# Galtvam/OthelloZero

Measured on NVIDIA B200. Metric: mcts_sims_per_sec, higher is better.
Workload: dtype bf16

## Files before the change

### othellozero_b200/csrc/oz_net.cu

```cuda
#include <cuda.h>
#include <cuda_bf16.h>
#include <stdlib.h>

#include "oz_engine.cuh"

typedef __nv_bfloat16 bf16;

namespace {

constexpr int BLOCK_M = 128;
constexpr int BLOCK_K = 64;
constexpr int UMMA_K = 16;
constexpr int STAGES = 4;
constexpr int A_STAGE_BYTES = BLOCK_M * BLOCK_K * 2;
constexpr int GEMM_THREADS = 256;
constexpr int EPI_RELU_BF16 = 0;
constexpr int EPI_HEADS = 1;
constexpr int EPI_LINEAR_BF16 = 2;
constexpr int N_PATTERNS = 19683;

struct GemmParams {
    int num_kb;
    int chunks_per_tap;
    int ntaps_x;
    int pad;
    int nb;
    int rows_per_board;
    int rows_valid;
    int split;
    int halves;
    int half_rows;
    int half_h;
    int tile_den;
    int tile_num;
    int n_tiles;
    int ldc;
    int max_count;
    unsigned long long* trace;
    unsigned a_bytes;
    const int* count;
    const float* bias;
    bf16* out;
    float* pi; float* logits; float* v;
    int nsq;
    const int* cache_idx; float* cache_pi; float* cache_v; unsigned long long* cache_tags;
};

__device__ __forceinline__ uint32_t smem_u32(const void* p) { return (uint32_t)__cvta_generic_to_shared(p); }

__device__ __forceinline__ void mbar_init(uint32_t bar, uint32_t count) {
    asm volatile("mbarrier.init.shared::cta.b64 [%0], %1;" ::"r"(bar), "r"(count) : "memory");
}
__device__ __forceinline__ void mbar_expect_tx(uint32_t bar, uint32_t bytes) {
    asm volatile("mbarrier.arrive.expect_tx.shared::cta.b64 _, [%0], %1;" ::"r"(bar), "r"(bytes) : "memory");
}
__device__ __forceinline__ void mbar_arrive(uint32_t bar) {
    asm volatile("mbarrier.arrive.shared::cta.b64 _, [%0];" ::"r"(bar) : "memory");
}
__device__ __forceinline__ bool mbar_try_wait(uint32_t bar, uint32_t parity) {
    uint32_t ok;
    asm volatile(
        "{\n\t.reg .pred p;\n\t"
        "mbarrier.try_wait.parity.shared::cta.b64 p, [%1], %2;\n\t"
        "selp.u32 %0, 1, 0, p;\n\t}"
        : "=r"(ok) : "r"(bar), "r"(parity) : "memory");
    return ok != 0;
}
__device__ __noinline__ void mbar_wait_slow(uint32_t bar, uint32_t parity) {
    unsigned long long t0 = 0;
    uint32_t spins = 0;
    while (!mbar_try_wait(bar, parity)) {
        if ((++spins & 255u) == 0) {
            unsigned long long t;
            asm volatile("mov.u64 %0, %%globaltimer;" : "=l"(t));
            if (t0 == 0) t0 = t;
            else if (t - t0 > 4000000000ull) __trap();
        }
    }
// ... 349 lines not shown
__device__ __forceinline__ void tma_load_4d_2sm(uint32_t dst, const CUtensorMap* m, uint32_t bar, int c0, int c1, int c2, int c3) {
    asm volatile(
        "cp.async.bulk.tensor.4d.cta_group::2.shared::cluster.global.mbarrier::complete_tx::bytes [%0], [%1, {%3, %4, %5, %6}], [%2];"
        ::"r"(dst), "l"(m), "r"(bar), "r"(c0), "r"(c1), "r"(c2), "r"(c3) : "memory");
}
__device__ __forceinline__ void tma_load_2d_2sm(uint32_t dst, const CUtensorMap* m, uint32_t bar, int c0, int c1) {
    asm volatile(
        "cp.async.bulk.tensor.2d.cta_group::2.shared::cluster.global.mbarrier::complete_tx::bytes [%0], [%1, {%3, %4}], [%2];"
        ::"r"(dst), "l"(m), "r"(bar), "r"(c0), "r"(c1) : "memory");
}
__device__ __forceinline__ void tmem_alloc_2sm(uint32_t dst_smem, uint32_t cols) {
    asm volatile("tcgen05.alloc.cta_group::2.sync.aligned.shared::cta.b32 [%0], %1;" ::"r"(dst_smem), "r"(cols) : "memory");
}
__device__ __forceinline__ void tmem_relinquish_2sm() {
    asm volatile("tcgen05.relinquish_alloc_permit.cta_group::2.sync.aligned;" ::: "memory");
}
__device__ __forceinline__ void tmem_dealloc_2sm(uint32_t taddr, uint32_t cols) {
    asm volatile("tcgen05.dealloc.cta_group::2.sync.aligned.b32 %0, %1;" ::"r"(taddr), "r"(cols) : "memory");
}
__device__ __forceinline__ void umma_bf16_2sm_lo(uint32_t d_tmem, uint32_t a_lo, uint32_t b_lo, uint32_t idesc, uint32_t accumulate) {
    asm volatile(
        "{\n\t.reg .pred p;\n\t.reg .b64 da, db;\n\t"
        "setp.ne.b32 p, %4, 0;\n\t"
        "mov.b64 da, {%1, %5};\n\t"
        "mov.b64 db, {%2, %5};\n\t"
        "tcgen05.mma.cta_group::2.kind::f16 [%0], da, db, %3, p;\n\t}"
        ::"r"(d_tmem), "r"(a_lo), "r"(b_lo), "r"(idesc), "r"(accumulate), "r"(SW128_DESC_HI) : "memory");
}
__device__ __forceinline__ void umma_commit_2sm(uint32_t bar, uint16_t cta_mask) {
    asm volatile("tcgen05.commit.cta_group::2.mbarrier::arrive::one.shared::cluster.multicast::cluster.b64 [%0], %1;"
                 ::"r"(bar), "h"(cta_mask) : "memory");
}

constexpr int STAGES2 = 6;
constexpr int B2_STAGE_BYTES = 128 * BLOCK_K * 2;
struct Gemm2Smem {
    static constexpr int OFF_A = 0;
    static constexpr int OFF_B = STAGES2 * A_STAGE_BYTES;
    static constexpr int OFF_BAR = OFF_B + STAGES2 * B2_STAGE_BYTES;
    static constexpr int OFF_TMEM = OFF_BAR + (2 * STAGES2 + 4) * 8;
    static constexpr int OFF_BIAS = OFF_TMEM + 16;
    static constexpr int BYTES = OFF_BIAS + 2 * 256 * 4;
    static constexpr int DYN_BYTES = BYTES + 1024;
};

__global__ void __cluster_dims__(2, 1, 1) __launch_bounds__(GEMM_THREADS, 1)
oz_gemm2_kernel(const __grid_constant__ CUtensorMap mapA, const __grid_constant__ CUtensorMap mapA2,
                const __grid_constant__ CUtensorMap mapB, const GemmParams p) {
    using S = Gemm2Smem;
    constexpr int BLOCK_N = 256;
    constexpr uint32_t TMEM_COLS = 2 * BLOCK_N;
    extern __shared__ uint8_t smem_raw[];
    const uint32_t raw = smem_u32(smem_raw);
    const uint32_t base = (raw + 1023u) & ~1023u;
    uint8_t* gbase = smem_raw + (base - raw);
    const uint32_t sA = base + S::OFF_A, sB = base + S::OFF_B, sBar = base + S::OFF_BAR;
    auto full_bar = [&](int s) { return sBar + 8u * s; };
    auto empty_bar = [&](int s) { return sBar + 8u * (STAGES2 + s); };
    auto tfull_bar = [&](int a) { return sBar + 8u * (2 * STAGES2 + a); };
    auto tempty_bar = [&](int a) { return sBar + 8u * (2 * STAGES2 + 2 + a); };
    volatile uint32_t* s_tmem = (volatile uint32_t*)(gbase + S::OFF_TMEM);
    float* s_bias = (float*)(gbase + S::OFF_BIAS);

    const int warp = threadIdx.x >> 5, lane = threadIdx.x & 31;
    const uint32_t rank = cluster_ctarank();
    const int cluster_id = blockIdx.x >> 1, num_clusters = gridDim.x >> 1;
    trace_begin(p.trace);
    int L = *p.count;
    if (L > p.max_count) L = p.max_count;
    const int m_tiles = (L * p.tile_num + p.tile_den - 1) / p.tile_den;
    const int num_pair_tiles = ((m_tiles + 1) >> 1) * p.n_tiles;

    if (warp == 0 && lane == 0) {
        tma_prefetch_desc(&mapA);
        tma_prefetch_desc(&mapB);
    }
    if (warp == 1 && lane == 0) {
// ... 67 lines not shown
                const uint32_t d_tmem = tmem_base + (uint32_t)(acc * BLOCK_N);
                for (int kb = 0; kb < p.num_kb; ++kb) {
                    mbar_wait(full_bar(stage), phase);
                    tc_fence_after();
                    const uint32_t a_lo = a_lo0 + (uint32_t)stage * (A_STAGE_BYTES >> 4);
                    const uint32_t b_lo = b_lo0 + (uint32_t)stage * (B2_STAGE_BYTES >> 4);
                    if (elect_one()) {
#pragma unroll
                        for (int k = 0; k < BLOCK_K / UMMA_K; ++k)
                            umma_bf16_2sm_lo(d_tmem, a_lo + 2u * k, b_lo + 2u * k, idesc, (kb | k) ? 1u : 0u);
                        umma_commit_2sm(empty_bar(stage), 3);
                    }
                    __syncwarp();
                    if (++stage == STAGES2) { stage = 0; phase ^= 1u; }
                }
                if (elect_one()) umma_commit_2sm(tfull_bar(acc), 3);
                __syncwarp();
                if (++acc == 2) { acc = 0; acc_phase ^= 1u; }
            }
        }
        __syncwarp();
    } else if (warp >= 4) {
        const int ew = warp - 4;
        const int et = threadIdx.x - 128;
        int acc = 0; uint32_t acc_phase = 0;
        for (int pt = cluster_id; pt < num_pair_tiles; pt += num_clusters) {
            const int m_pair = pt / p.n_tiles, n_idx = pt - m_pair * p.n_tiles;
            const int m_tile = 2 * m_pair + (int)rank;
            float* bias = s_bias + acc * BLOCK_N;
            for (int i = et; i < BLOCK_N; i += 128) bias[i] = p.bias[n_idx * BLOCK_N + i];
            epi_bar_sync();
            mbar_wait(tfull_bar(acc), acc_phase);
            tc_fence_after();
            const int r = ew * 32 + lane;
            const long long grow = (long long)m_tile * p.rows_valid + r;
            const bool ok = (r < p.rows_valid) && (grow < (long long)L * p.rows_per_board);
            const uint32_t t_row = tmem_base + (uint32_t)(acc * BLOCK_N) + ((uint32_t)(ew * 32) << 16);
            bf16* orow = p.out + grow * p.ldc + (long long)n_idx * BLOCK_N;
#pragma unroll 1
            for (int c = 0; c < BLOCK_N / 32; ++c) {
                uint32_t v[32];
                tmem_ld32(t_row + (uint32_t)(c * 32), v);
                tmem_ld_wait();
                if (ok) {
                    uint32_t packed[16];
#pragma unroll
                    for (int j = 0; j < 16; ++j) {
                        const float2 bj = *reinterpret_cast<const float2*>(bias + c * 32 + 2 * j);
                        const float2 y = __fadd2_rn(make_float2(__uint_as_float(v[2 * j]), __uint_as_float(v[2 * j + 1])), bj);
                        packed[j] = pack_relu_bf16x2(y.x, y.y);
                    }
                    uint4* dst = reinterpret_cast<uint4*>(orow + c * 32);
#pragma unroll
                    for (int q = 0; q < 4; ++q)
                        dst[q] = make_uint4(packed[4 * q], packed[4 * q + 1], packed[4 * q + 2], packed[4 * q + 3]);
                }
            }
            tc_fence_before();
            __syncwarp();
            if (lane == 0) mbar_arrive_cluster(mapa_cluster(tempty_bar(acc), 0));
            if (++acc == 2) { acc = 0; acc_phase ^= 1u; }
        }
    }
    __syncwarp();
    tc_fence_before();
    __syncthreads();
    cluster_sync_all();
    if (warp == 2) {
        tc_fence_after();
        tmem_dealloc_2sm(tmem_base, TMEM_COLS);
    }
    trace_end(p.trace);
}

constexpr int TSTAGES = 3;
constexpr int T_B_STAGE_BYTES = 256 * BLOCK_K * 2;
struct TailSmem {
    static constexpr int OFF_A = 0;
    static constexpr int OFF_B = TSTAGES * A_STAGE_BYTES;
    static constexpr int OFF_F2 = OFF_B + TSTAGES * T_B_STAGE_BYTES;
    static constexpr int OFF_BAR = OFF_F2 + 4 * A_STAGE_BYTES;
    static constexpr int OFF_TMEM = OFF_BAR + (2 * TSTAGES + 7) * 8 + 8;
    static constexpr int OFF_BIAS = OFF_TMEM + 16;
    static constexpr int BYTES = OFF_BIAS + 640 * 4;
    static constexpr int DYN_BYTES = BYTES + 1024;
};
struct TailParams {
    int max_count;
    const int* count;
    const float* bias4; const float* bias5;
    bf16* f2;
    float* pi; float* logits; float* v;
    int nsq;
    const int* cache_idx; float* cache_pi; float* cache_v; unsigned long long* cache_tags;
    unsigned long long* trace;
    unsigned long long* dbg;
};

__global__ void __launch_bounds__(GEMM_THREADS, 1)
oz_tail_kernel(const __grid_constant__ CUtensorMap mapA ,
               const __grid_constant__ CUtensorMap mapB4 ,
               const __grid_constant__ CUtensorMap mapB5 , const TailParams p) {
    using S = TailSmem;
// ... 723 lines not shown
            Wt[(size_t)o * K + k] = __float2bfloat16(tile[threadIdx.x][i] * s);
        }
    }
    if (blockIdx.x == 0 && threadIdx.y == 0) {
        int o = o0 + threadIdx.x;
        if (o < Nout) {
            float s = gamma ? gamma[o] / sqrtf(var[o] + eps) : 1.0f;
            bias_out[o] = gamma ? (b[o] - mean[o]) * s + beta[o] : b[o];
        }
    }
}

typedef CUresult (*PFN_tmapEncodeTiled)(CUtensorMap*, CUtensorMapDataType, cuuint32_t, void*, const cuuint64_t*,
                                        const cuuint64_t*, const cuuint32_t*, const cuuint32_t*, CUtensorMapInterleave,
                                        CUtensorMapSwizzle, CUtensorMapL2promotion, CUtensorMapFloatOOBfill);

PFN_tmapEncodeTiled get_encode_fn() {
    static PFN_tmapEncodeTiled fn = nullptr;
    if (!fn) {
        void* p = nullptr;
        cudaDriverEntryPointQueryResult q;
        if (cudaGetDriverEntryPoint("cuTensorMapEncodeTiled", &p, cudaEnableDefault, &q) == cudaSuccess &&
            q == cudaDriverEntryPointSuccess)
            fn = (PFN_tmapEncodeTiled)p;
    }
    return fn;
}

}

struct OzLayer {
    CUtensorMap mapA, mapA2, mapB, mapB2;
    bool use_2sm = false;
    GemmParams p;
    int block_n;
    int epi;
    int max_tiles;
    double flops_per_board;
};

struct OzNet {
    int n = 0, C = 0, Bmax = 0;
    bool loaded = false;
    bool timing = false;
    bool pdl = true;
    int timing_every = 16;
    long forwards = 0;
    int sm_count = 148;
    bf16* table1 = nullptr;
    bool conv2_table = true;
    bf16* table2 = nullptr; bf16* w2perm = nullptr; float* zero_bias = nullptr; int* d_npat = nullptr;
    OzLayer tbl;
    bool conv3_wino = false;
    bool fused_tail = false;
    bf16* v3 = nullptr;
    bf16* u3 = nullptr;
    CUtensorMap mapV, mapU;
    WinoParams wp;
    unsigned long long* trace = nullptr;
    int trace_slots = 0, trace_next = 0;
    char trace_name[256][12];
    bf16 *w[6] = {nullptr}; float* bias[6] = {nullptr};
    bf16 *act1 = nullptr, *act2 = nullptr, *act3 = nullptr, *act4 = nullptr, *f1 = nullptr, *f2 = nullptr;
    OzLayer layer[6];
    static constexpr int RING = 8;
    cudaEvent_t ev[RING][8] = {{nullptr}};
    bool ev_used[RING] = {false};
    int ev_next = 0;
    double ms_sum[8] = {0};
    long ms_cnt = 0;
    void* allocs[32];
    int n_allocs = 0;
};

static void oz_net_harvest(OzNet* net, int r) {
    cudaEventSynchronize(net->ev[r][7]);
    for (int i = 0; i < 7; ++i) {
        float ms = 0.f;
// ... 3 lines not shown
    net->ev_used[r] = false;
}

static int net_alloc(OzNet* net, void** p, size_t bytes) {
    cudaError_t err = cudaMalloc(p, bytes + 256);
    if (err != cudaSuccess) { oz_set_error("cudaMalloc(%zu) failed: %s", bytes, cudaGetErrorString(err)); return OZ_ERR_NOMEM; }
    net->allocs[net->n_allocs++] = *p;
    return OZ_OK;
}

int64_t oz_net_blob_floats_impl(int n, int C) {
    if ((n != 6 && n != 8) || C <= 0) return -1;
    int64_t nsq = n * n, k1 = (int64_t)(n - 4) * (n - 4) * C;
    int64_t t = 0;
    t += 18LL * C + C + 4LL * C;
    t += 3 * (9LL * C * C + C + 4LL * C);
    t += k1 * 1024 + 1024 + 4 * 1024;
    t += 1024LL * 512 + 512 + 4 * 512;
    t += 512 * nsq + nsq;
    t += 512 + 1;
    return t;
}

int oz_net_create(oz_engine* e) {
    e->net = nullptr;
    if (e->cfg.prior_mode != OZ_PRIOR_NET) return OZ_OK;
    OzNet* net = new OzNet();
    net->n = e->cfg.board_size;
    net->Bmax = e->cfg.max_games * (e->cfg.vl_width > 1 ? e->cfg.vl_width : 1);
    const char* t = getenv("OZ_NET_TIMING");
    net->timing = t && t[0] == '1';
    const char* pd = getenv("OZ_NET_NO_PDL");
    net->pdl = !(pd && pd[0] == '1');
    const char* c2 = getenv("OZ_NET_CONV2");
    net->conv2_table = !(c2 && c2[0] == 'g');
    const char* c3 = getenv("OZ_NET_CONV3");
    net->conv3_wino = net->conv2_table && c3 && c3[0] == 'w';
    const char* tl = getenv("OZ_NET_TAIL");
    net->fused_tail = tl && tl[0] == 'f';
    const char* tr = getenv("OZ_NET_TRACE");
    if (tr && atoi(tr) > 0) net->trace_slots = atoi(tr) > 256 ? 256 : atoi(tr);
    const char* te = getenv("OZ_NET_TIMING_EVERY");
    if (te && atoi(te) > 0) net->timing_every = atoi(te);
    int dev = e->cfg.device;
    cudaDeviceGetAttribute(&net->sm_count, cudaDevAttrMultiProcessorCount, dev);
    for (int r = 0; r < OzNet::RING; ++r)
        for (int i = 0; i < 8; ++i) cudaEventCreate(&net->ev[r][i]);
    e->net = net;
    return OZ_OK;
}

static unsigned long long* trace_slot(OzNet* net, const char* name) {
    if (!net->trace || net->trace_next >= net->trace_slots) return nullptr;
    snprintf(net->trace_name[net->trace_next], sizeof(net->trace_name[0]), "%s", name);
    return net->trace + 2 * (net->trace_next++);
}

static void trace_dump(OzNet* net) {
    if (!net->trace || net->trace_next == 0) return;
    cudaDeviceSynchronize();
    unsigned long long* h = (unsigned long long*)malloc(sizeof(unsigned long long) * 2 * net->trace_next);
    cudaMemcpy(h, net->trace, sizeof(unsigned long long) * 2 * net->trace_next, cudaMemcpyDeviceToHost);
    unsigned long long t0 = ~0ull;
    for (int i = 0; i < net->trace_next; ++i) if (h[2 * i] < t0) t0 = h[2 * i];
    for (int i = 0; i < net->trace_next; ++i)
        fprintf(stderr, "OZ_TRACE %3d %-8s start %9.1f us  end %9.1f us  dur %8.1f us\n", i, net->trace_name[i],
                (h[2 * i] - t0) / 1e3, (h[2 * i + 1] - t0) / 1e3, (h[2 * i + 1] - h[2 * i]) / 1e3);
    free(h);
}

void oz_net_destroy(oz_engine* e) {
    OzNet* net = e->net;
    if (!net) return;
    trace_dump(net);
    for (int i = 0; i < net->n_allocs; ++i) cudaFree(net->allocs[i]);
    for (int r = 0; r < OzNet::RING; ++r)
        for (int i = 0; i < 8; ++i) if (net->ev[r][i]) cudaEventDestroy(net->ev[r][i]);
    delete net;
    e->net = nullptr;
}

static int make_map_A(CUtensorMap* m, bf16* base, int Cdim, int W, int H, int B, int bw, int bh, int nb) {
    PFN_tmapEncodeTiled enc = get_encode_fn();
    if (!enc) { oz_set_error("cuTensorMapEncodeTiled entry point not available"); return OZ_ERR_CUDA; }
    cuuint64_t dims[4] = {(cuuint64_t)Cdim, (cuuint64_t)W, (cuuint64_t)H, (cuuint64_t)B};
    cuuint64_t strides[3] = {(cuuint64_t)Cdim * 2, (cuuint64_t)Cdim * 2 * W, (cuuint64_t)Cdim * 2 * W * H};
    cuuint32_t box[4] = {(cuuint32_t)BLOCK_K, (cuuint32_t)bw, (cuuint32_t)bh, (cuuint32_t)nb};
    cuuint32_t estr[4] = {1, 1, 1, 1};
    CUresult r = enc(m, CU_TENSOR_MAP_DATA_TYPE_BFLOAT16, 4, base, dims, strides, box, estr, CU_TENSOR_MAP_INTERLEAVE_NONE,
                     CU_TENSOR_MAP_SWIZZLE_128B, CU_TENSOR_MAP_L2_PROMOTION_L2_256B, CU_TENSOR_MAP_FLOAT_OOB_FILL_NONE);
    if (r != CUDA_SUCCESS) { oz_set_error("cuTensorMapEncodeTiled(A) failed: %d", (int)r); return OZ_ERR_CUDA; }
    return OZ_OK;
}

static int make_map_B(CUtensorMap* m, bf16* base, int K, int Nout, int block_n) {
    PFN_tmapEncodeTiled enc = get_encode_fn();
    if (!enc) { oz_set_error("cuTensorMapEncodeTiled entry point not available"); return OZ_ERR_CUDA; }
    cuuint64_t dims[2] = {(cuuint64_t)K, (cuuint64_t)Nout};
    cuuint64_t strides[1] = {(cuuint64_t)K * 2};
// ... 19 lines not shown
    p.rows_valid = nb * rows_per_board;
    p.tile_num = 1;
    p.tile_den = nb;
    static const bool allow_split = !(getenv("OZ_NET_NO_SPLIT") && getenv("OZ_NET_NO_SPLIT")[0] == '1');
    if (allow_split && ntaps == 3 && (oh % 2) == 0 && (BLOCK_M - nb * rows_per_board) * 2 >= rows_per_board) {
        p.split = 1;
        p.half_h = oh / 2;
        p.half_rows = (oh / 2) * ow;
        p.halves = 2 * nb + 1;
        p.rows_valid = p.halves * p.half_rows;
        p.tile_num = 2;
        p.tile_den = p.halves;
    }
    p.ntaps_x = ntaps;
    p.pad = pad;
    p.chunks_per_tap = cin / BLOCK_K;
    p.num_kb = ntaps * ntaps * p.chunks_per_tap;
    p.n_tiles = nout_pad / block_n;
    p.ldc = ldc;
    p.max_count = bmax;
    p.a_bytes = (unsigned)(p.rows_valid * BLOCK_K * 2);
    p.bias = bias;
    p.out = out;
    p.nsq = net->n * net->n;
    Lr.block_n = block_n;
    Lr.epi = epi;
    Lr.max_tiles = ((bmax * p.tile_num + p.tile_den - 1) / p.tile_den) * p.n_tiles;
    int rc = make_map_A(&Lr.mapA, in, cin, iw, ih, bmax, ow, oh, nb);
    if (rc) return rc;
    rc = make_map_A(&Lr.mapA2, in, cin, iw, ih, bmax, ow, p.split ? oh / 2 : oh, p.split ? 1 : nb);
    if (rc) return rc;
    static const bool allow_2sm = !(getenv("OZ_NET_NO_2SM") && getenv("OZ_NET_NO_2SM")[0] == '1');
    Lr.use_2sm = allow_2sm && epi == EPI_RELU_BF16 && block_n == 256;
    if (Lr.use_2sm) {
        rc = make_map_B(&Lr.mapB2, weights, ntaps * ntaps * cin, nout_pad, 128);
        if (rc) return rc;
    }
    return make_map_B(&Lr.mapB, weights, ntaps * ntaps * cin, nout_pad, block_n);
}

int oz_net_load(oz_engine* e, const float* blob, int64_t n_floats, int channels, bool on_device) {
    OzNet* net = e->net;
    if (!net) { oz_set_error("engine was not created with OZ_PRIOR_NET"); return OZ_ERR_STATE; }
    const int n = net->n, C = channels, nsq = n * n, B = net->Bmax;
    OZ_REQUIRE(C >= 128 && C % 128 == 0 && C <= 1024, "channels must be a multiple of 128 in [128,1024] (got %d)", C);
    const int64_t need = oz_net_blob_floats_impl(n, C);
    OZ_REQUIRE(n_floats == need, "weight blob has %lld floats, expected %lld", (long long)n_floats, (long long)need);
    if (net->loaded && net->C != C) { oz_set_error("channel count cannot change after the first load"); return OZ_ERR_STATE; }
    cudaStream_t st = e->stream;
    const int o2 = n - 2, o4 = n - 4;
    const int K1 = o4 * o4 * C;
    int rc;
    if (!net->loaded) {
        net->C = C;
        const size_t kc = 9ull * C * C;
#define NA(ptr, bytes) if ((rc = net_alloc(net, (void**)&(ptr), (bytes)))) return rc;
        NA(net->table1, (size_t)N_PATTERNS * C * 2)
        NA(net->w[0], kc * 2) NA(net->w[1], kc * 2) NA(net->w[2], kc * 2)
        NA(net->w[3], (size_t)K1 * 1024 * 2) NA(net->w[4], 1024ull * 512 * 2) NA(net->w[5], 128ull * 512 * 2)
        NA(net->bias[0], C * 4) NA(net->bias[1], C * 4) NA(net->bias[2], C * 4)
        NA(net->bias[3], 1024 * 4) NA(net->bias[4], 512 * 4) NA(net->bias[5], 128 * 4)
        NA(net->act1, (size_t)B * nsq * C * 2)
        if (!net->conv3_wino) NA(net->act2, (size_t)B * nsq * C * 2)
        NA(net->act3, (size_t)B * o2 * o2 * C * 2) NA(net->act4, (size_t)B * o4 * o4 * C * 2)
        NA(net->f1, (size_t)B * 1024 * 2) NA(net->f2, (size_t)B * 512 * 2)
        if (net->trace_slots) {
// ... 31 lines not shown
            wp.n_tiles = C / WINO_N;
            wp.C = C;
            wp.bmax = B;
            wp.max_count = B;
            wp.a_bytes = (unsigned)(wp.rows_valid * BLOCK_K * 2);
            wp.bias = net->bias[1];
            wp.out = net->act3;
            if ((rc = make_map_A(&net->mapV, net->v3, C, n, T, 4 * B, o2, T, wp.nb))) return rc;
            if ((rc = make_map_B(&net->mapU, net->u3, 3 * C, 4 * C, WINO_N / 2))) return rc;
            OZ_CUDA(cudaFuncSetAttribute(oz_wino_kernel, cudaFuncAttributeMaxDynamicSharedMemorySize, WinoSmem::DYN_BYTES));
        }
        if (net->conv2_table) {
            if ((rc = setup_layer(net, net->tbl, net->w2perm, net->zero_bias, N_PATTERNS, net->table1, C, 1, 1, 1, 1, 1, 0,
                                  9 * C, 256, EPI_LINEAR_BF16, net->table2, 9 * C))) return rc;
            OZ_CUDA(cudaFuncSetAttribute(oz_gemm_kernel<256, EPI_LINEAR_BF16>, cudaFuncAttributeMaxDynamicSharedMemorySize,
                                         GemmSmem<256>::DYN_BYTES));
            OZ_CUDA(cudaFuncSetAttribute(oz_gemm_kernel<128, EPI_LINEAR_BF16>, cudaFuncAttributeMaxDynamicSharedMemorySize,
                                         GemmSmem<128>::DYN_BYTES));
            OZ_CUDA(cudaFuncSetAttribute(oz_gemm_kernel<128, EPI_LINEAR_BF16>, cudaFuncAttributeMaxDynamicSharedMemorySize,
                                         GemmSmem<128>::DYN_BYTES));
            OZ_CUDA(cudaMemsetAsync(net->table2 + (size_t)N_PATTERNS * 9 * C, 0, 9ull * C * 2, st));
            OZ_CUDA(cudaMemsetAsync(net->zero_bias, 0, 9ull * C * 4, st));
            const int npat = N_PATTERNS;
            OZ_CUDA(cudaMemcpyAsync(net->d_npat, &npat, sizeof(int), cudaMemcpyHostToDevice, st));
            OZ_CUDA(cudaStreamSynchronize(st));
        }
        OZ_CUDA(cudaFuncSetAttribute(oz_gemm_kernel<256, EPI_RELU_BF16>, cudaFuncAttributeMaxDynamicSharedMemorySize,
                                     GemmSmem<256>::DYN_BYTES));
        OZ_CUDA(cudaFuncSetAttribute(oz_gemm_kernel<128, EPI_HEADS>, cudaFuncAttributeMaxDynamicSharedMemorySize,
                                     GemmSmem<128>::DYN_BYTES));
        OZ_CUDA(cudaFuncSetAttribute(oz_gemm_kernel<128, EPI_RELU_BF16>, cudaFuncAttributeMaxDynamicSharedMemorySize,
                                     GemmSmem<128>::DYN_BYTES));
        OZ_CUDA(cudaFuncSetAttribute(oz_gemm2_kernel, cudaFuncAttributeMaxDynamicSharedMemorySize, Gemm2Smem::DYN_BYTES));
        OZ_CUDA(cudaFuncSetAttribute(oz_tail_kernel, cudaFuncAttributeMaxDynamicSharedMemorySize, TailSmem::DYN_BYTES));
        OZ_CUDA(cudaMemsetAsync(net->w[5], 0, 128ull * 512 * 2, st));
        OZ_CUDA(cudaMemsetAsync(net->bias[5], 0, 128 * 4, st));
    }
    const float* d = blob;
    struct Staged {
        float* p = nullptr;
        cudaStream_t st;
        ~Staged() { if (p) { cudaStreamSynchronize(st); cudaFree(p); } }
    } staged;
    staged.st = st;
    if (!on_device) {
        OZ_CUDA(cudaMalloc((void**)&staged.p, (size_t)need * 4));
        OZ_CUDA(cudaMemcpyAsync(staged.p, blob, (size_t)need * 4, cudaMemcpyHostToDevice, st));
        d = staged.p;
    }
    const float eps = 1e-3f;
    const float* q = d;
    auto take = [&](int64_t cnt) { const float* r = q; q += cnt; return r; };
    dim3 tb(32, 8);
    {
        const float* w1 = take(18LL * C); const float* b1 = take(C);
        const float* g = take(C); const float* be = take(C); const float* mu = take(C); const float* va = take(C);
        conv1_table_kernel<<<N_PATTERNS, 256, 0, st>>>(w1, b1, g, be, mu, va, eps, C, net->table1);
        OZ_CUDA(cudaGetLastError());
        e->launches++;
    }
    for (int li = 0; li < 3; ++li) {
        const int K = 9 * C;
        const float* w = take((int64_t)K * C); const float* b = take(C);
        const float* g = take(C); const float* be = take(C); const float* mu = take(C); const float* va = take(C);
        fold_weights_kernel<<<dim3((K + 31) / 32, (C + 31) / 32), tb, 0, st>>>(w, b, g, be, mu, va, eps, K, C, net->w[li], net->bias[li]);
        OZ_CUDA(cudaGetLastError());
// ... 77 lines not shown
    }
    if (tm) cudaEventRecord(ev[1], st);
    if (net->conv2_table) {
        int blocks = max_count < net->sm_count * 2 ? max_count : net->sm_count * 2;
        const bf16* t2 = net->table2; const float* b2 = net->bias[0];
        unsigned long long* ts = trace_slot(net, "gather");
#define OZ_T2K(NJ, W, X, OUT) conv2_table_gather_kernel<NJ, W, X><<<blocks, 256, 0, st>>>(own_dev, opp_dev, count_dev, max_count, n, C, t2, b2, OUT, net->Bmax, ts)
#define OZ_T2(NJ)                                                                  \
    if (net->conv3_wino) { if (C == 256 * NJ) OZ_T2K(NJ, true, true, net->v3); else OZ_T2K(NJ, true, false, net->v3); } \
    else { if (C == 256 * NJ) OZ_T2K(NJ, false, true, net->act2); else OZ_T2K(NJ, false, false, net->act2); }
        switch (C / 256) {
            case 0: case 1: OZ_T2(1); break;
            case 2: OZ_T2(2); break;
            case 3: OZ_T2(3); break;
            default: OZ_T2(4); break;
        }
#undef OZ_T2
#undef OZ_T2K
        OZ_CUDA(cudaGetLastError());
        e->launches++;
        if (tm) cudaEventRecord(ev[2], st);
    }
    for (int li = net->conv2_table ? 1 : 0; li < 6; ++li) {
        OzLayer& Lr = net->layer[li];
        GemmParams p = Lr.p;
        p.count = count_dev;
        p.max_count = max_count;
        static const char* lname[6] = {"conv2", "conv3", "conv4", "fc1", "fc2", "heads"};
        if (li == 5 && net->fused_tail) {
            if (tm) cudaEventRecord(ev[2 + li], st);
            continue;
        }
        p.trace = (li == 4 && net->fused_tail) ? nullptr : trace_slot(net, lname[li]);
        p.pi = pi_dev; p.logits = logits_dev; p.v = v_dev;
        if (publish && li == 5) {
            p.cache_idx = e->tp.leaf_cache_idx; p.cache_pi = e->tp.cache_pi; p.cache_v = e->tp.cache_v;
            p.cache_tags = e->tp.cache_tags;
        }
        int tiles = ((max_count * p.tile_num + p.tile_den - 1) / p.tile_den) * p.n_tiles;
        int grid = tiles < net->sm_count ? tiles : net->sm_count;
        if (grid < 1) grid = 1;
        cudaLaunchAttribute attr[1];
        attr[0].id = cudaLaunchAttributeProgrammaticStreamSerialization;
        attr[0].val.programmaticStreamSerializationAllowed = 1;
        cudaLaunchConfig_t cfg{};
        cfg.blockDim = dim3(GEMM_THREADS);
        cfg.stream = st;
        cfg.attrs = attr;
        cfg.numAttrs = net->pdl ? 1 : 0;
        cudaError_t lerr;
        if (li == 4 && net->fused_tail) {
            TailParams tp{};
            tp.max_count = max_count;
            tp.count = count_dev;
            tp.bias4 = net->bias[4]; tp.bias5 = net->bias[5];
            tp.f2 = net->f2;
            tp.pi = pi_dev; tp.logits = logits_dev; tp.v = v_dev;
            tp.nsq = nsq;
            if (publish) {
                tp.cache_idx = e->tp.leaf_cache_idx; tp.cache_pi = e->tp.cache_pi; tp.cache_v = e->tp.cache_v;
                tp.cache_tags = e->tp.cache_tags;
            }
            tp.trace = trace_slot(net, "fc2+heads");
            if (tp.trace && net->trace_next + 4 <= net->trace_slots) {
                tp.dbg = trace_slot(net, "t:w,f0"); trace_slot(net, "t:r0,f1"); trace_slot(net, "t:r1,f2"); trace_slot(net, "t:lg,end");
            }
            const int m_tiles = (max_count + BLOCK_M - 1) / BLOCK_M;
            cfg.gridDim = dim3(m_tiles < net->sm_count ? (m_tiles < 1 ? 1 : m_tiles) : net->sm_count);
            cfg.dynamicSmemBytes = TailSmem::DYN_BYTES;
            lerr = cudaLaunchKernelEx(&cfg, oz_tail_kernel, Lr.mapA, Lr.mapB, net->layer[5].mapB, tp);
        } else if (li == 1 && net->conv3_wino) {
            WinoParams wp = net->wp;
            wp.count = count_dev;
            wp.max_count = max_count;
            wp.trace = p.trace;
            const int m_tiles = (max_count + wp.nb - 1) / wp.nb;
            const int pairs = ((m_tiles + 1) / 2) * wp.n_tiles;
            int g2 = 2 * pairs < (net->sm_count & ~1) ? 2 * pairs : (net->sm_count & ~1);
            if (g2 < 2) g2 = 2;
            cfg.blockDim = dim3(WINO_THREADS);
            cfg.gridDim = dim3(g2);
            cfg.dynamicSmemBytes = WinoSmem::DYN_BYTES;
            lerr = cudaLaunchKernelEx(&cfg, oz_wino_kernel, net->mapV, net->mapU, wp);
        } else if (Lr.use_2sm) {
            int m_tiles = (max_count * p.tile_num + p.tile_den - 1) / p.tile_den;
            int pairs = ((m_tiles + 1) / 2) * p.n_tiles;
            int g2 = 2 * pairs < (net->sm_count & ~1) ? 2 * pairs : (net->sm_count & ~1);
            if (g2 < 2) g2 = 2;
            cfg.gridDim = dim3(g2);
            cfg.dynamicSmemBytes = Gemm2Smem::DYN_BYTES;
            lerr = cudaLaunchKernelEx(&cfg, oz_gemm2_kernel, Lr.mapA, Lr.mapA2, Lr.mapB2, p);
        } else if (Lr.epi == EPI_RELU_BF16 && Lr.block_n == 256) {
            cfg.gridDim = dim3(grid);
            cfg.dynamicSmemBytes = GemmSmem<256>::DYN_BYTES;
            lerr = cudaLaunchKernelEx(&cfg, oz_gemm_kernel<256, EPI_RELU_BF16>, Lr.mapA, Lr.mapA2, Lr.mapB, p);
        } else if (Lr.epi == EPI_RELU_BF16) {
            cfg.gridDim = dim3(grid);
            cfg.dynamicSmemBytes = GemmSmem<128>::DYN_BYTES;
            lerr = cudaLaunchKernelEx(&cfg, oz_gemm_kernel<128, EPI_RELU_BF16>, Lr.mapA, Lr.mapA2, Lr.mapB, p);
        } else {
            cfg.gridDim = dim3(grid);
            cfg.dynamicSmemBytes = GemmSmem<128>::DYN_BYTES;
            lerr = cudaLaunchKernelEx(&cfg, oz_gemm_kernel<128, EPI_HEADS>, Lr.mapA, Lr.mapA2, Lr.mapB, p);
        }
        OZ_CUDA(lerr);
        OZ_CUDA(cudaGetLastError());
        e->launches++;
        if (tm) cudaEventRecord(ev[2 + li], st);
    }
    return OZ_OK;
}

void oz_net_set_timing_impl(oz_engine* e, bool on) {
    if (e->net) e->net->timing = on;
}

int oz_net_times(oz_engine* e, float* ms8) {
    OzNet* net = e->net;
    for (int i = 0; i < 8; ++i) ms8[i] = 0.f;
    if (!net) return OZ_OK;
    for (int r = 0; r < OzNet::RING; ++r)
        if (net->ev_used[r]) oz_net_harvest(net, r);
    if (net->ms_cnt > 0)
        for (int i = 0; i < 7; ++i) ms8[i] = (float)(net->ms_sum[i] / (double)net->ms_cnt);
// ... 28 lines not shown
```

Before: 4.780 million.

## Add wide 512-column SM-pair GEMM kernel and smem-staged coalesced epilogue stores

Adds an opt-in (OZ_NET_WIDE=1) 2-SM cluster GEMM kernel that computes 512 output columns per M-pair, so each A tile loaded from memory feeds two accumulators. It uses eight epilogue warps and falls back to 256-wide items for the leftover tiles to keep clusters balanced. Separately, the default 2-SM kernel's epilogue now stages each warp's rows through swizzled shared memory so a warp writes whole row segments together instead of each lane writing its own row. The staging adds extra shared traffic and warp syncs per 32-column chunk, and the wide path is off by default.

```diff
diff --git a/othellozero_b200/csrc/oz_net.cu b/othellozero_b200/csrc/oz_net.cu
--- a/othellozero_b200/csrc/oz_net.cu
+++ b/othellozero_b200/csrc/oz_net.cu
@@ -44,6 +44,7 @@
     float* pi; float* logits; float* v;
     int nsq;
     const int* cache_idx; float* cache_pi; float* cache_v; unsigned long long* cache_tags;
+    unsigned long long* stall;
 };
 
 __device__ __forceinline__ uint32_t smem_u32(const void* p) { return (uint32_t)__cvta_generic_to_shared(p); }
@@ -459,6 +460,22 @@
                  ::"r"(bar), "h"(cta_mask) : "memory");
 }
 
+constexpr int EPI_STAGE_BYTES = 32 * 64;
+__device__ __forceinline__ void warp_store_rows(uint4* stage, const uint32_t (&pk)[16], bf16* base, int ldc, int lim, int lane) {
+    const int sw = (lane >> 1) & 3;
+#pragma unroll
+    for (int q = 0; q < 4; ++q) stage[lane * 4 + (q ^ sw)] = make_uint4(pk[4 * q], pk[4 * q + 1], pk[4 * q + 2], pk[4 * q + 3]);
+    __syncwarp();
+    const int q = lane & 3;
+#pragma unroll
+    for (int j = 0; j < 4; ++j) {
+        const int r = j * 8 + (lane >> 2);
+        const uint4 v = stage[r * 4 + (q ^ ((r >> 1) & 3))];
+        if (r < lim) *reinterpret_cast<uint4*>(base + (long long)r * ldc + q * 8) = v;
+    }
+    __syncwarp();
+}
+
 constexpr int STAGES2 = 6;
 constexpr int B2_STAGE_BYTES = 128 * BLOCK_K * 2;
 struct Gemm2Smem {
@@ -467,9 +484,11 @@
     static constexpr int OFF_BAR = OFF_B + STAGES2 * B2_STAGE_BYTES;
     static constexpr int OFF_TMEM = OFF_BAR + (2 * STAGES2 + 4) * 8;
     static constexpr int OFF_BIAS = OFF_TMEM + 16;
-    static constexpr int BYTES = OFF_BIAS + 2 * 256 * 4;
+    static constexpr int OFF_STAGE = OFF_BIAS + 2 * 256 * 4;
+    static constexpr int BYTES = OFF_STAGE + 4 * EPI_STAGE_BYTES;
     static constexpr int DYN_BYTES = BYTES + 1024;
 };
+static_assert(Gemm2Smem::DYN_BYTES <= 227 * 1024, "SM-pair ring exceeds the shared memory of one CTA");
 
 __global__ void __cluster_dims__(2, 1, 1) __launch_bounds__(GEMM_THREADS, 1)
 oz_gemm2_kernel(const __grid_constant__ CUtensorMap mapA, const __grid_constant__ CUtensorMap mapA2,
@@ -603,29 +622,25 @@
             epi_bar_sync();
             mbar_wait(tfull_bar(acc), acc_phase);
             tc_fence_after();
-            const int r = ew * 32 + lane;
-            const long long grow = (long long)m_tile * p.rows_valid + r;
-            const bool ok = (r < p.rows_valid) && (grow < (long long)L * p.rows_per_board);
+            const long long g0 = (long long)m_tile * p.rows_valid + ew * 32;
+            const long long live = (long long)L * p.rows_per_board - g0;
+            const int lim = (int)(live < p.rows_valid - ew * 32 ? live : p.rows_valid - ew * 32);
             const uint32_t t_row = tmem_base + (uint32_t)(acc * BLOCK_N) + ((uint32_t)(ew * 32) << 16);
-            bf16* orow = p.out + grow * p.ldc + (long long)n_idx * BLOCK_N;
+            bf16* obase = p.out + g0 * p.ldc + (long long)n_idx * BLOCK_N;
+            uint4* stage = reinterpret_cast<uint4*>(gbase + S::OFF_STAGE + ew * EPI_STAGE_BYTES);
 #pragma unroll 1
             for (int c = 0; c < BLOCK_N / 32; ++c) {
                 uint32_t v[32];
                 tmem_ld32(t_row + (uint32_t)(c * 32), v);
                 tmem_ld_wait();
-                if (ok) {
-                    uint32_t packed[16];
-#pragma unroll
-                    for (int j = 0; j < 16; ++j) {
-                        const float2 bj = *reinterpret_cast<const float2*>(bias + c * 32 + 2 * j);
-                        const float2 y = __fadd2_rn(make_float2(__uint_as_float(v[2 * j]), __uint_as_float(v[2 * j + 1])), bj);
-                        packed[j] = pack_relu_bf16x2(y.x, y.y);
-                    }
-                    uint4* dst = reinterpret_cast<uint4*>(orow + c * 32);
-#pragma unroll
-                    for (int q = 0; q < 4; ++q)
-                        dst[q] = make_uint4(packed[4 * q], packed[4 * q + 1], packed[4 * q + 2], packed[4 * q + 3]);
-                }
+                uint32_t packed[16];
+#pragma unroll
+                for (int j = 0; j < 16; ++j) {
+                    const float2 bj = *reinterpret_cast<const float2*>(bias + c * 32 + 2 * j);
+                    const float2 y = __fadd2_rn(make_float2(__uint_as_float(v[2 * j]), __uint_as_float(v[2 * j + 1])), bj);
+                    packed[j] = pack_relu_bf16x2(y.x, y.y);
+                }
+                warp_store_rows(stage, packed, obase + c * 32, p.ldc, lim, lane);
             }
             tc_fence_before();
             __syncwarp();
@@ -640,6 +655,274 @@
     if (warp == 2) {
         tc_fence_after();
         tmem_dealloc_2sm(tmem_base, TMEM_COLS);
+    }
+    trace_end(p.trace);
+}
+
+constexpr int STAGESW = 4;
+constexpr int GEMMW_THREADS = 384;
+struct GemmWSmem {
+    static constexpr int B_STAGE_BYTES = 2 * B2_STAGE_BYTES;
+    static constexpr int OFF_A = 0;
+    static constexpr int OFF_B = STAGESW * A_STAGE_BYTES;
+    static constexpr int OFF_BAR = OFF_B + STAGESW * B_STAGE_BYTES;
+    static constexpr int OFF_TMEM = OFF_BAR + (2 * STAGESW + 4) * 8;
+    static constexpr int OFF_BIAS = OFF_TMEM + 16;
+    static constexpr int OFF_STAGE = OFF_BIAS + 2 * 512 * 4;
+    static constexpr int BYTES = OFF_STAGE + 8 * EPI_STAGE_BYTES;
+    static constexpr int DYN_BYTES = BYTES + 1024;
+};
+static_assert(GemmWSmem::DYN_BYTES <= 227 * 1024, "wide-tile ring exceeds the shared memory of one CTA");
+
+struct WideTile { int m_pair, n0; bool wide; };
+__device__ __forceinline__ WideTile wide_tile(int it, int n_wide, int nw) {
+    if (it < n_wide) {
+        const int mp = it / nw;
+        return {mp, (it - mp * nw) * 512, true};
+    }
+    const int w = n_wide + ((it - n_wide) >> 1), mp = w / nw;
+    return {mp, (w - mp * nw) * 512 + ((it - n_wide) & 1) * 256, false};
+}
+
+__global__ void __cluster_dims__(2, 1, 1) __launch_bounds__(GEMMW_THREADS, 1)
+oz_gemm2w_kernel(const __grid_constant__ CUtensorMap mapA, const __grid_constant__ CUtensorMap mapA2,
+                 const __grid_constant__ CUtensorMap mapB, const GemmParams p) {
+    using S = GemmWSmem;
+    constexpr uint32_t HALF_COLS = 256;
+    extern __shared__ uint8_t smem_raw[];
+    const uint32_t raw = smem_u32(smem_raw);
+    const uint32_t base = (raw + 1023u) & ~1023u;
+    uint8_t* gbase = smem_raw + (base - raw);
+    const uint32_t sA = base + S::OFF_A, sB = base + S::OFF_B, sBar = base + S::OFF_BAR;
+    auto full_bar = [&](int s) { return sBar + 8u * s; };
+    auto empty_bar = [&](int s) { return sBar + 8u * (STAGESW + s); };
+    auto tfull_bar = [&](int a) { return sBar + 8u * (2 * STAGESW + a); };
+    auto tempty_bar = [&](int a) { return sBar + 8u * (2 * STAGESW + 2 + a); };
+    volatile uint32_t* s_tmem = (volatile uint32_t*)(gbase + S::OFF_TMEM);
+    float* s_bias = (float*)(gbase + S::OFF_BIAS);
+
+    const int warp = threadIdx.x >> 5, lane = threadIdx.x & 31;
+    const uint32_t rank = cluster_ctarank();
+    const int cluster_id = blockIdx.x >> 1, num_clusters = gridDim.x >> 1;
+    trace_begin(p.trace);
+    int L = *p.count;
+    if (L > p.max_count) L = p.max_count;
+    const int m_tiles = (L * p.tile_num + p.tile_den - 1) / p.tile_den;
+    const int nw = p.n_tiles >> 1;
+    const int all_wide = ((m_tiles + 1) >> 1) * nw;
+    const int n_wide = all_wide - all_wide % num_clusters;
+    const int num_items = n_wide + 2 * (all_wide - n_wide);
+
+    if (warp == 0 && lane == 0) {
+        tma_prefetch_desc(&mapA);
+        tma_prefetch_desc(&mapB);
+    }
+    if (warp == 1 && lane == 0) {
+        for (int s = 0; s < STAGESW; ++s) { mbar_init(full_bar(s), 1); mbar_init(empty_bar(s), 1); }
+        for (int a = 0; a < 2; ++a) { mbar_init(tfull_bar(a), 1); mbar_init(tempty_bar(a), 16); }
+        fence_barrier_init();
+        fence_proxy_async();
+    }
+    if (warp == 2) {
+        tmem_alloc_2sm(smem_u32((const void*)s_tmem), 2 * HALF_COLS);
+        tmem_relinquish_2sm();
+    }
+    tc_fence_before();
+    __syncthreads();
+    cluster_sync_all();
+    tc_fence_after();
+    const uint32_t tmem_base = *s_tmem;
+    pdl_launch_dependents();
+
+    if (warp == 0) {
+        {
+            pdl_wait();
+            int stage = 0; uint32_t phase = 0;
+            const int ntaps_y = p.num_kb / (p.chunks_per_tap * p.ntaps_x);
+            const uint32_t off_main_after_half = (uint32_t)(p.half_rows * 128);
+            const uint32_t off_half_after_main = (uint32_t)(p.nb * p.rows_per_board * 128);
+            const uint32_t fb0 = mapa_cluster(full_bar(0), 0);
+            for (int it = cluster_id; it < num_items; it += num_clusters) {
+                const WideTile t = wide_tile(it, n_wide, nw);
+                const int m_tile = 2 * t.m_pair + (int)rank;
+                const int nB = t.n0 + (int)rank * 128;
+                const uint32_t tx_bytes = 2u * (p.a_bytes + (t.wide ? 2u : 1u) * (unsigned)B2_STAGE_BYTES);
+                const int hb0 = m_tile * p.halves;
+                const bool odd = p.split && (hb0 & 1);
+                const int bA = p.split ? ((hb0 >> 1) + (odd ? 1 : 0)) : m_tile * p.nb;
+                const int bH = (hb0 >> 1) + (odd ? 0 : p.nb);
+                const uint32_t offA = odd ? off_main_after_half : 0u;
+                const uint32_t offH = odd ? 0u : off_half_after_main;
+                const int yH = odd ? p.half_h : 0;
+                int kcol = 0;
+                for (int ky = -p.pad; ky < ntaps_y - p.pad; ++ky) {
+                    for (int kx = -p.pad; kx < p.ntaps_x - p.pad; ++kx) {
+                        for (int c0 = 0; c0 < p.chunks_per_tap * BLOCK_K; c0 += BLOCK_K) {
+                            mbar_wait(empty_bar(stage), phase ^ 1u);
+                            if (elect_one()) {
+                                const uint32_t fb = fb0 + 8u * (uint32_t)stage;
+                                if (rank == 0) mbar_expect_tx(full_bar(stage), tx_bytes);
+                                const uint32_t dstA = sA + stage * A_STAGE_BYTES;
+                                tma_load_4d_2sm(dstA + offA, &mapA, fb, c0, kx, ky, bA);
+                                if (p.split) tma_load_4d_2sm(dstA + offH, &mapA2, fb, c0, kx, ky + yH, bH);
+                                const uint32_t dstB = sB + stage * S::B_STAGE_BYTES;
+                                tma_load_2d_2sm(dstB, &mapB, fb, kcol, nB);
+                                if (t.wide) tma_load_2d_2sm(dstB + B2_STAGE_BYTES, &mapB, fb, kcol, nB + 256);
+                            }
+                            __syncwarp();
+                            kcol += BLOCK_K;
+                            if (++stage == STAGESW) { stage = 0; phase ^= 1u; }
+                        }
+                    }
+                }
+            }
+        }
+        __syncwarp();
+    } else if (warp == 1) {
+        if (rank == 0) {
+            constexpr uint32_t idesc = make_idesc(256, HALF_COLS);
+            const uint32_t a_lo0 = sw128_desc_lo(sA), b_lo0 = sw128_desc_lo(sB);
+            int stage = 0; uint32_t phase = 0;
+            uint32_t ph0 = 0, ph1 = 0;
+            int acc = 0;
+            unsigned long long stall_ns = 0;
+            auto wait_drained = [&](int a, uint32_t parity) {
+                const unsigned long long t0 = p.stall ? global_ns() : 0ull;
+                mbar_wait(tempty_bar(a), parity);
+                tc_fence_after();
+                if (p.stall) stall_ns += global_ns() - t0;
+            };
+            auto mma_kblock = [&](int s, int h, int a, int kb) {
+                const uint32_t a_lo = a_lo0 + (uint32_t)s * (A_STAGE_BYTES >> 4);
+                const uint32_t b_lo = b_lo0 + (uint32_t)s * (S::B_STAGE_BYTES >> 4) + (uint32_t)h * (B2_STAGE_BYTES >> 4);
+                const uint32_t d_tmem = tmem_base + (uint32_t)a * HALF_COLS;
+#pragma unroll
+                for (int k = 0; k < BLOCK_K / UMMA_K; ++k)
+                    umma_bf16_2sm_lo(d_tmem, a_lo + 2u * k, b_lo + 2u * k, idesc, (kb | k) ? 1u : 0u);
+            };
+            for (int it = cluster_id; it < num_items; it += num_clusters) {
+                const WideTile t = wide_tile(it, n_wide, nw);
+                if (t.wide) {
+                    wait_drained(0, ph0 ^ 1u);
+                    const int lead = p.num_kb < STAGESW ? p.num_kb : STAGESW;
+                    int s1 = stage;
+                    for (int kb = 0; kb < lead; ++kb) {
+                        mbar_wait(full_bar(stage), phase);
+                        tc_fence_after();
+                        if (elect_one()) {
+                            mma_kblock(stage, 0, 0, kb);
+                            if (kb == p.num_kb - 1) umma_commit_2sm(tfull_bar(0), 3);
+                        }
+                        __syncwarp();
+                        if (++stage == STAGESW) { stage = 0; phase ^= 1u; }
+                    }
+                    wait_drained(1, ph1 ^ 1u);
+                    for (int kb = 0; kb < lead; ++kb) {
+                        if (elect_one()) {
+                            mma_kblock(s1, 1, 1, kb);
+                            umma_commit_2sm(empty_bar(s1), 3);
+                        }
+                        __syncwarp();
+                        if (++s1 == STAGESW) s1 = 0;
+                    }
+                    for (int kb = lead; kb < p.num_kb; ++kb) {
+                        mbar_wait(full_bar(stage), phase);
+                        tc_fence_after();
+                        if (elect_one()) {
+                            mma_kblock(stage, 0, 0, kb);
+                            if (kb == p.num_kb - 1) umma_commit_2sm(tfull_bar(0), 3);
+                            mma_kblock(stage, 1, 1, kb);
+                            umma_commit_2sm(empty_bar(stage), 3);
+                        }
+                        __syncwarp();
+                        if (++stage == STAGESW) { stage = 0; phase ^= 1u; }
+                    }
+                    if (elect_one()) umma_commit_2sm(tfull_bar(1), 3);
+                    __syncwarp();
+                    ph0 ^= 1u; ph1 ^= 1u;
+                } else {
+                    wait_drained(acc, (acc ? ph1 : ph0) ^ 1u);
+                    for (int kb = 0; kb < p.num_kb; ++kb) {
+                        mbar_wait(full_bar(stage), phase);
+                        tc_fence_after();
+                        if (elect_one()) {
+                            mma_kblock(stage, 0, acc, kb);
+                            umma_commit_2sm(empty_bar(stage), 3);
+                        }
+                        __syncwarp();
+                        if (++stage == STAGESW) { stage = 0; phase ^= 1u; }
+                    }
+                    if (elect_one()) umma_commit_2sm(tfull_bar(acc), 3);
+                    __syncwarp();
+                    if (acc) ph1 ^= 1u; else ph0 ^= 1u;
+                    acc ^= 1;
+                }
+            }
+            if (p.stall && lane == 0) {
+                atomicAdd(p.stall, stall_ns);
+                atomicAdd(p.stall + 1, (unsigned long long)(n_wide / num_clusters));
+            }
+        }
+        __syncwarp();
+    } else if (warp >= 4) {
+        const int ew = warp & 3;
+        const int colh = (warp - 4) >> 2;
+        const int et = threadIdx.x - 128;
+        uint32_t ph0 = 0, ph1 = 0;
+        int acc = 0, buf = 0;
+        for (int it = cluster_id; it < num_items; it += num_clusters) {
+            const WideTile t = wide_tile(it, n_wide, nw);
+            const int m_tile = 2 * t.m_pair + (int)rank;
+            float* bias = s_bias + buf * 512;
+            for (int i = et; i < (t.wide ? 512 : 256); i += 256) bias[i] = p.bias[t.n0 + i];
+            asm volatile("bar.sync 1, 256;" ::: "memory");
+            const long long g0 = (long long)m_tile * p.rows_valid + ew * 32;
+            const long long live = (long long)L * p.rows_per_board - g0;
+            const int lim = (int)(live < p.rows_valid - ew * 32 ? live : p.rows_valid - ew * 32);
+            const uint32_t t_row = tmem_base + ((uint32_t)(ew * 32) << 16) + (uint32_t)(colh * 128);
+            bf16* obase = p.out + g0 * p.ldc + t.n0 + colh * 128;
+            uint4* stage = reinterpret_cast<uint4*>(gbase + S::OFF_STAGE + (warp - 4) * EPI_STAGE_BYTES);
+            auto drain = [&](int a, uint32_t parity, int h) {
+                mbar_wait(tfull_bar(a), parity);
+                tc_fence_after();
+                const float* bh = bias + h * 256 + colh * 128;
+#pragma unroll 1
+                for (int c = 0; c < 4; ++c) {
+                    uint32_t v[32];
+                    tmem_ld32(t_row + (uint32_t)a * HALF_COLS + (uint32_t)(c * 32), v);
+                    tmem_ld_wait();
+                    uint32_t packed[16];
+#pragma unroll
+                    for (int j = 0; j < 16; ++j) {
+                        const float2 bj = *reinterpret_cast<const float2*>(bh + c * 32 + 2 * j);
+                        const float2 y = __fadd2_rn(make_float2(__uint_as_float(v[2 * j]), __uint_as_float(v[2 * j + 1])), bj);
+                        packed[j] = pack_relu_bf16x2(y.x, y.y);
+                    }
+                    warp_store_rows(stage, packed, obase + h * 256 + c * 32, p.ldc, lim, lane);
+                }
+                tc_fence_before();
+                __syncwarp();
+                if (lane == 0) mbar_arrive_cluster(mapa_cluster(tempty_bar(a), 0));
+            };
+            if (t.wide) {
+                drain(0, ph0, 0);
+                drain(1, ph1, 1);
+                ph0 ^= 1u; ph1 ^= 1u;
+            } else {
+                drain(acc, acc ? ph1 : ph0, 0);
+                if (acc) ph1 ^= 1u; else ph0 ^= 1u;
+                acc ^= 1;
+            }
+            buf ^= 1;
+        }
+    }
+    __syncwarp();
+    tc_fence_before();
+    __syncthreads();
+    cluster_sync_all();
+    if (warp == 2) {
+        tc_fence_after();
+        tmem_dealloc_2sm(tmem_base, 2 * HALF_COLS);
     }
     trace_end(p.trace);
 }
@@ -1429,6 +1712,7 @@
 struct OzLayer {
     CUtensorMap mapA, mapA2, mapB, mapB2;
     bool use_2sm = false;
+    bool use_wide = false;
     GemmParams p;
     int block_n;
     int epi;
@@ -1441,6 +1725,7 @@
     bool loaded = false;
     bool timing = false;
     bool pdl = true;
+    bool wide = false;
     int timing_every = 16;
     long forwards = 0;
     int sm_count = 148;
@@ -1510,6 +1795,8 @@
     net->timing = t && t[0] == '1';
     const char* pd = getenv("OZ_NET_NO_PDL");
     net->pdl = !(pd && pd[0] == '1');
+    const char* wd = getenv("OZ_NET_WIDE");
+    net->wide = wd && wd[0] == '1';
     const char* c2 = getenv("OZ_NET_CONV2");
     net->conv2_table = !(c2 && c2[0] == 'g');
     const char* c3 = getenv("OZ_NET_CONV3");
@@ -1540,9 +1827,12 @@
     unsigned long long* h = (unsigned long long*)malloc(sizeof(unsigned long long) * 2 * net->trace_next);
     cudaMemcpy(h, net->trace, sizeof(unsigned long long) * 2 * net->trace_next, cudaMemcpyDeviceToHost);
     unsigned long long t0 = ~0ull;
-    for (int i = 0; i < net->trace_next; ++i) if (h[2 * i] < t0) t0 = h[2 * i];
+    for (int i = 0; i < net->trace_next; ++i) if (net->trace_name[i][0] != '~' && h[2 * i] < t0) t0 = h[2 * i];
     for (int i = 0; i < net->trace_next; ++i)
-        fprintf(stderr, "OZ_TRACE %3d %-8s start %9.1f us  end %9.1f us  dur %8.1f us\n", i, net->trace_name[i],
+        if (net->trace_name[i][0] == '~')
+            fprintf(stderr, "OZ_TRACE %3d %-8s MMA warps waited %8.1f us for drained accumulators over %llu wide tiles\n", i,
+                    net->trace_name[i], (double)(h[2 * i] + 1) / 1e3, h[2 * i + 1]);
+        else fprintf(stderr, "OZ_TRACE %3d %-8s start %9.1f us  end %9.1f us  dur %8.1f us\n", i, net->trace_name[i],
                 (h[2 * i] - t0) / 1e3, (h[2 * i + 1] - t0) / 1e3, (h[2 * i + 1] - h[2 * i]) / 1e3);
     free(h);
 }
@@ -1628,6 +1918,7 @@
     if (rc) return rc;
     static const bool allow_2sm = !(getenv("OZ_NET_NO_2SM") && getenv("OZ_NET_NO_2SM")[0] == '1');
     Lr.use_2sm = allow_2sm && epi == EPI_RELU_BF16 && block_n == 256;
+    Lr.use_wide = Lr.use_2sm && net->wide && ntaps == 3 && nout_pad % 512 == 0;
     if (Lr.use_2sm) {
         rc = make_map_B(&Lr.mapB2, weights, ntaps * ntaps * cin, nout_pad, 128);
         if (rc) return rc;
@@ -1725,6 +2016,7 @@
         OZ_CUDA(cudaFuncSetAttribute(oz_gemm_kernel<128, EPI_RELU_BF16>, cudaFuncAttributeMaxDynamicSharedMemorySize,
                                      GemmSmem<128>::DYN_BYTES));
         OZ_CUDA(cudaFuncSetAttribute(oz_gemm2_kernel, cudaFuncAttributeMaxDynamicSharedMemorySize, Gemm2Smem::DYN_BYTES));
+        OZ_CUDA(cudaFuncSetAttribute(oz_gemm2w_kernel, cudaFuncAttributeMaxDynamicSharedMemorySize, GemmWSmem::DYN_BYTES));
         OZ_CUDA(cudaFuncSetAttribute(oz_tail_kernel, cudaFuncAttributeMaxDynamicSharedMemorySize, TailSmem::DYN_BYTES));
         OZ_CUDA(cudaMemsetAsync(net->w[5], 0, 128ull * 512 * 2, st));
         OZ_CUDA(cudaMemsetAsync(net->bias[5], 0, 128 * 4, st));
@@ -1868,6 +2160,7 @@
             continue;
         }
         p.trace = (li == 4 && net->fused_tail) ? nullptr : trace_slot(net, lname[li]);
+        if (p.trace && Lr.use_wide) p.stall = trace_slot(net, "~drain");
         p.pi = pi_dev; p.logits = logits_dev; p.v = v_dev;
         if (publish && li == 5) {
             p.cache_idx = e->tp.leaf_cache_idx; p.cache_pi = e->tp.cache_pi; p.cache_v = e->tp.cache_v;
@@ -1924,8 +2217,14 @@
             int g2 = 2 * pairs < (net->sm_count & ~1) ? 2 * pairs : (net->sm_count & ~1);
             if (g2 < 2) g2 = 2;
             cfg.gridDim = dim3(g2);
-            cfg.dynamicSmemBytes = Gemm2Smem::DYN_BYTES;
-            lerr = cudaLaunchKernelEx(&cfg, oz_gemm2_kernel, Lr.mapA, Lr.mapA2, Lr.mapB2, p);
+            if (Lr.use_wide) {
+                cfg.blockDim = dim3(GEMMW_THREADS);
+                cfg.dynamicSmemBytes = GemmWSmem::DYN_BYTES;
+                lerr = cudaLaunchKernelEx(&cfg, oz_gemm2w_kernel, Lr.mapA, Lr.mapA2, Lr.mapB2, p);
+            } else {
+                cfg.dynamicSmemBytes = Gemm2Smem::DYN_BYTES;
+                lerr = cudaLaunchKernelEx(&cfg, oz_gemm2_kernel, Lr.mapA, Lr.mapA2, Lr.mapB2, p);
+            }
         } else if (Lr.epi == EPI_RELU_BF16 && Lr.block_n == 256) {
             cfg.gridDim = dim3(grid);
             cfg.dynamicSmemBytes = GemmSmem<256>::DYN_BYTES;
```

Result: no change. 4.824 million, median of 6 (+0.9%).
